# ethz-tb/orcAI

Measured on AMD Instinct MI355X. Metric: audio_seconds_per_s, higher is better.
Workload: dtype f32; 1 GPU; orcai-V1 predict, 1 h synthetic recording @48 kHz, 1833 snippets; parallelism=independent recordings x1

## Files before the change

orcai_amd/csrc/model_fwd.hip:

```cpp
#include <hip/hip_runtime.h>
#include <type_traits>

#include <cstdint>

#include "lds_dma.h"
#include "orcai_hip.h"
#include "zero_fill.h"

__attribute__((visibility("hidden"))) int lstm_wide_fwd_launch(const float* xz, const float* Uw, int B, int T, int units, float* out, float* gates, float* cstate, void* stream);

int g_orcai_lstm_split = 1;

namespace {

typedef float f32x4 __attribute__((ext_vector_type(4)));

__device__ __forceinline__ f32x4 mfma16(float a, float b, f32x4 c) { return __builtin_amdgcn_mfma_f32_16x16x4f32(a, b, c, 0, 0, 0); }


__device__ __forceinline__ void xcd_remap(int& bx, int& by) {
  const unsigned nbx = gridDim.x, total = nbx * gridDim.y;
  const unsigned L = blockIdx.y * nbx + blockIdx.x;
  const unsigned k = L & 7u, q = total >> 3, r = total & 7u;
  const unsigned Lp = k * q + (k < r ? k : r) + (L >> 3);
// ... 1572 lines not shown
#pragma unroll
      for (int m = 0; m < MT; ++m) acc[m][t] = mfma16(afrag[m], d[t], acc[m][t]);
  }

#pragma unroll
  for (int t = 0; t < 4; ++t) {
#pragma unroll
    for (int m = 0; m < MT; ++m) {
      const int oq = m * 4 + lk;
      const int e0 = VERT ? 2 * t : 3 * t;
      float mx[4] = {v[e0][m].x, v[e0][m].y, v[e0][m].z, v[e0][m].w};
#pragma unroll
      for (int dy = 1; dy < 3; ++dy) {
        mx[0] = fmaxf(mx[0], v[e0 + dy][m].x); mx[1] = fmaxf(mx[1], v[e0 + dy][m].y);
        mx[2] = fmaxf(mx[2], v[e0 + dy][m].z); mx[3] = fmaxf(mx[3], v[e0 + dy][m].w);
      }
      if (oidx[t] >= 0 && oq < CQ) {
        float o[4];
#pragma unroll
        for (int r = 0; r < 4; ++r) o[r] = (oq * 4 + r < C) ? mx[r] + (acc[m][t][r] + br_r[m][r]) : 0.0f;
        if (!SCATTER) {
          reinterpret_cast<float4*>(out)[((int64_t)b * CQ + oq) * plane_o + oidx[t]] = make_float4(o[0], o[1], o[2], o[3]);
        } else {
          const int orow = oidx[t] / WPo - R, ocol = oidx[t] - (orow + R) * WPo;
          const int rr = rm.base + b * rm.img_step + orow;
          if ((orow >= rm.r_lo || rr == orow) && orow < rm.r_hi) {
            const float4 val = make_float4(o[0], o[1], o[2], o[3]);
#pragma unroll
            for (int fi = 0; fi < kRowFamilies; ++fi) {
              if (fi >= rm.nfam) break;
              const RowFamily& fm = rm.f[fi];
              const int rel = rr - fm.offset - fm.keep_lo;
              if (rel < 0) continue;
              const int jhi = rel / fm.period;
              const int64_t plane_d = (int64_t)(fm.Hd + 2 * R) * WPo;
#pragma unroll
              for (int d = 0; d < 2; ++d) {
                const int j = jhi - d, y = rr - fm.offset - j * fm.period;
                if (j >= 0 && j < fm.count && y < fm.keep_hi)
                  reinterpret_cast<float4*>(fm.out)[((int64_t)j * CQ + oq) * plane_d + (int64_t)(y + R) * WPo + ocol] = val;
              }
            }
          }
        }
      }
    }
    if (t + DEPTH < 4) {
      load_tile(t + DEPTH);
      __builtin_amdgcn_sched_barrier(0);
    }
  }
}

constexpr int GP = 128 + 16;

constexpr int GBK = 32;

__global__ __launch_bounds__(256) void gemm_kernel(const float* __restrict__ A, const float* __restrict__ Bm, const float* __restrict__ bias,
                                                    const float* __restrict__ scale, const float* __restrict__ shift, float* __restrict__ C,
                                                    int M, int N, int K, int act, int vec) {
  __shared__ __attribute__((aligned(16))) float As[GBK][GP];
  __shared__ __attribute__((aligned(16))) float Bs[GBK][GP];
  const int tid = threadIdx.x, lane = tid & 63, wave = tid >> 6;
  const int wm = wave >> 1, wn = wave & 1;
  const int lk = lane >> 4, lj = lane & 15;
  const int64_t m0 = (int64_t)blockIdx.y * 128;
  const int n0 = blockIdx.x * 128;
  f32x4 acc[4][4];
#pragma unroll
  for (int i = 0; i < 4; ++i)
#pragma unroll
    for (int j = 0; j < 4; ++j) acc[i][j] = (f32x4){0.f, 0.f, 0.f, 0.f};

  float4 ra[4], rb[4];
  auto fetch = [&](int k0) {
#pragma unroll
    for (int g = 0; g < 4; ++g) {
      const int f = tid + 256 * g;
      {
        const int64_t m = m0 + (f & 127);
        const int k = k0 + (f >> 7) * 4;
        float v[4] = {0.f, 0.f, 0.f, 0.f};
        if (m < M) {
          const float* p = A + m * K + k;
          if (vec && k + 3 < K) {
            const float4 t = *reinterpret_cast<const float4*>(p);
            v[0] = t.x; v[1] = t.y; v[2] = t.z; v[3] = t.w;
          } else {
#pragma unroll
            for (int e = 0; e < 4; ++e) v[e] = (k + e < K) ? p[e] : 0.0f;
          }
        }
        ra[g] = make_float4(v[0], v[1], v[2], v[3]);
      }
      {
        const int k = k0 + (f >> 5), n = n0 + (f & 31) * 4;
        float v[4] = {0.f, 0.f, 0.f, 0.f};
        if (k < K) {
          const float* p = Bm + (int64_t)k * N + n;
          if (vec && n + 3 < N) {
            const float4 t = *reinterpret_cast<const float4*>(p);
            v[0] = t.x; v[1] = t.y; v[2] = t.z; v[3] = t.w;
          } else {
#pragma unroll
            for (int e = 0; e < 4; ++e) v[e] = (n + e < N) ? p[e] : 0.0f;
          }
        }
        rb[g] = make_float4(v[0], v[1], v[2], v[3]);
      }
    }
  };
  fetch(0);
  for (int k0 = 0; k0 < K; k0 += GBK) {
    __syncthreads();
#pragma unroll
    for (int g = 0; g < 4; ++g) {
      const int f = tid + 256 * g;
      const int m = f & 127, k = (f >> 7) * 4;
      As[k][m] = ra[g].x; As[k + 1][m] = ra[g].y; As[k + 2][m] = ra[g].z; As[k + 3][m] = ra[g].w;
      *reinterpret_cast<float4*>(&Bs[f >> 5][(f & 31) * 4]) = rb[g];
    }
    __syncthreads();
    if (k0 + GBK < K) fetch(k0 + GBK);
#pragma unroll
    for (int kk = 0; kk < GBK / 4; ++kk) {
      float a[4], bq[4];
#pragma unroll
      for (int i = 0; i < 4; ++i) a[i] = As[kk * 4 + lk][wm * 64 + i * 16 + lj];
#pragma unroll
      for (int j = 0; j < 4; ++j) bq[j] = Bs[kk * 4 + lk][wn * 64 + j * 16 + lj];
#pragma unroll
      for (int i = 0; i < 4; ++i)
#pragma unroll
        for (int j = 0; j < 4; ++j) acc[i][j] = mfma16(a[i], bq[j], acc[i][j]);
    }
  }
#pragma unroll
  for (int i = 0; i < 4; ++i)
#pragma unroll
    for (int r = 0; r < 4; ++r) {
      const int64_t m = m0 + wm * 64 + i * 16 + lk * 4 + r;
      if (m >= M) continue;
#pragma unroll
      for (int j = 0; j < 4; ++j) {
        const int n = n0 + wn * 64 + j * 16 + lj;
        if (n >= N) continue;
        float v = acc[i][j][r] + (bias ? bias[n] : 0.0f);
        if (act == 1) v = fmaxf(v, 0.0f);
        if (scale) v = fmaf(v, scale[n], shift[n]);
        C[m * N + n] = v;
      }
    }
}

__device__ __forceinline__ float sigmoidf_(float x) { return __builtin_amdgcn_rcpf(1.0f + __expf(-x)); }
__device__ __forceinline__ float tanhf_(float x) { return fmaf(-2.0f, __builtin_amdgcn_rcpf(__expf(2.0f * x) + 1.0f), 1.0f); }

__device__ __forceinline__ float dpp_xor8(float v) {
  return __uint_as_float(__builtin_amdgcn_update_dpp(0u, __float_as_uint(v), 0x128 , 0xf, 0xf, true));
}
template <class StoreState>
__device__ __forceinline__ void lstm_gate_stage(const float (&z0)[4], const float (&z1)[4], float (&cst)[4], int lj, StoreState store_state) {
  const bool low = lj < 8;
  const float m1 = low ? 2.0f : -1.0f;
  float a0[4], a1[4];
#pragma unroll
  for (int r = 0; r < 4; ++r) {
    a0[r] = sigmoidf_(z0[r]);
    const float rc = __builtin_amdgcn_rcpf(__expf(m1 * z1[r]) + 1.0f);
    a1[r] = low ? fmaf(-2.0f, rc, 1.0f) : rc;
  }
#pragma unroll
  for (int j = 0; j < 2; ++j) {
    const float got0 = dpp_xor8(low ? a0[2 + j] : a0[j]), got1 = dpp_xor8(low ? a1[2 + j] : a1[j]);
    const float gi = low ? a0[j] : got0, gf = low ? got0 : a0[2 + j];
    const float gg = low ? a1[j] : got1, go = low ? got1 : a1[2 + j];
    const float c = gf * cst[j] + gi * gg;
    const float h = go * tanhf_(c);
    cst[j] = c;
    store_state(low ? j : 2 + j, h);
  }
}

template <int U>
__global__ __launch_bounds__(U * 8) void lstm_kernel(const float* __restrict__ xz , const float* __restrict__ Uw ,
                                                      int B, int T, float* __restrict__ out ) {
  constexpr int KSTEPS = U / 4, HP = U + 2;
  __shared__ float hbuf[2][16][HP];
  const int tid = threadIdx.x, lane = tid & 63, wave = tid >> 6;
  const int lk = lane >> 4, lj = lane & 15;
  const int dir = blockIdx.y;
  const int b0 = blockIdx.x * 16;
  const float* Ud = Uw + (int64_t)dir * U * 4 * U;

  float ufrag[2][KSTEPS];
#pragma unroll
  for (int nt = 0; nt < 2; ++nt)
#pragma unroll
    for (int kk = 0; kk < KSTEPS; ++kk) ufrag[nt][kk] = Ud[(int64_t)(kk * 4 + lk) * (4 * U) + wave * 32 + nt * 16 + lj];

  for (int i = tid; i < 2 * 16 * HP; i += U * 8) (&hbuf[0][0][0])[i] = 0.0f;
  float cst[4] = {0.f, 0.f, 0.f, 0.f};
  __syncthreads();

  const int unit = wave * 8 + (lj & 7);
// ... 774 lines not shown
    hipLaunchKernelGGL((pool_res_add_x_kernel<MT, true, true>), vgrid, dim3(256), 0, st, s, prev, C, Cp, H, W, WP, R, Ho, Wo, WPo, tot_h / 2, wr, br, out, compact, \
                       vtasks, mg, ntc, rm);                                                                                                                     \
  else                                                                                                                                                           \
    hipLaunchKernelGGL((pool_res_add_x_kernel<MT, false, true>), grid, dim3(256), 0, st, s, prev, C, Cp, H, W, WP, R, Ho, Wo, WPo, tot_h / 2, wr, br, out, compact, \
                       tasks, mg, 0, rm)
  switch ((C + 15) / 16) {
    case 1: ORCAI_POOL_SCATTER(1); break;
    case 2: ORCAI_POOL_SCATTER(2); break;
    case 3: ORCAI_POOL_SCATTER(3); break;
    case 4: ORCAI_POOL_SCATTER(4); break;
  }
#undef ORCAI_POOL_SCATTER
  return (int)hipGetLastError();
}

int orcai_pool_res_add_scatter(const float* s, const float* prev, int B, int C, int Cp, int H, int W, int ksize, const float* wr, const float* br, float* out,
                               int xpooled, int Hd, int nsnip, int period, int base, int img_step, int r_lo, int r_hi, int keep_lo, int keep_hi,
                               void* stream) {
  if (!s || !prev || !wr || !br || !out || B <= 0 || C <= 0 || Cp <= 0 || H <= 0 || W <= 0 || nsnip <= 0 || period <= 0) return ORCAI_E_BADARG;
  if (xpooled & ~3) return ORCAI_E_BADARG;
  if (keep_lo < 0 || keep_hi > Hd || keep_lo >= keep_hi || Hd != 2 * period || base < 0 || img_step < 0) return ORCAI_E_BADARG;
  RowMap rm{};
  rm.base = base;
  rm.img_step = img_step;
  rm.r_lo = r_lo;
  rm.r_hi = r_hi;
  rm.nfam = 1;
  rm.f[0] = RowFamily{out, Hd, period, 0, nsnip, keep_lo, keep_hi};
  return pool_res_scatter_launch(s, prev, B, C, Cp, H, W, ksize, wr, br, xpooled, rm, stream);
}

int orcai_pool_res_add_scatter_families(const float* s, const float* prev, int B, int C, int Cp, int H, int W, int ksize, const float* wr, const float* br,
                                        int xpooled, int base, int img_step, int r_lo, int r_hi, const orcai_row_family* fams, int nfam, void* stream) {
  if (!s || !prev || !wr || !br || !fams || B <= 0 || C <= 0 || Cp <= 0 || H <= 0 || W <= 0 || nfam <= 0) return ORCAI_E_BADARG;
  if ((xpooled & ~3) || base < 0 || img_step < 0) return ORCAI_E_BADARG;
  if (nfam > kRowFamilies) return ORCAI_E_UNSUPPORTED;
  RowMap rm{};
  rm.base = base;
  rm.img_step = img_step;
  rm.r_lo = r_lo;
  rm.r_hi = r_hi;
  rm.nfam = nfam;
  for (int i = 0; i < nfam; ++i) {
    const orcai_row_family& f = fams[i];
    if (!f.out || f.Hd <= 0 || f.period <= 0 || f.count <= 0 || f.offset < 0 || f.keep_lo < 0 || f.keep_hi > f.Hd || f.keep_lo >= f.keep_hi)
      return ORCAI_E_BADARG;
    if (f.keep_hi - f.keep_lo > 2 * f.period) return ORCAI_E_UNSUPPORTED;
    if ((int64_t)f.offset + (int64_t)(f.count - 1) * f.period + f.Hd >= (1ll << 31)) return ORCAI_E_UNSUPPORTED;
    rm.f[i] = RowFamily{f.out, f.Hd, f.period, f.offset, f.count, f.keep_lo, f.keep_hi};
  }
  return pool_res_scatter_launch(s, prev, B, C, Cp, H, W, ksize, wr, br, xpooled, rm, stream);
}

int orcai_gemm_bias_act(const float* A, const float* Bm, const float* bias, const float* scale, const float* shift, float* C, int64_t M, int N,
                        int K, int act, void* stream) {
  if (!A || !Bm || !C || M <= 0 || N <= 0 || K <= 0 || (scale && !shift)) return ORCAI_E_BADARG;
  dim3 grid((N + 127) / 128, (unsigned)((M + 127) / 128));
  const int vec = (((uintptr_t)A | (uintptr_t)Bm) % 16 == 0 && K % 4 == 0 && N % 4 == 0) ? 1 : 0;
  hipLaunchKernelGGL(gemm_kernel, grid, dim3(256), 0, (hipStream_t)stream, A, Bm, bias, scale, shift, C, (int)M, N, K, act, vec);
  return (int)hipGetLastError();
}

int orcai_lstm_split(int on) {
  const int prev = g_orcai_lstm_split;
  if (on >= 0) g_orcai_lstm_split = on ? 1 : 0;
  return prev;
}

int orcai_lstm_recurrent(const float* xz, const float* Uw, int B, int T, int units, float* out, void* stream) {
  if (!xz || !Uw || !out || B <= 0 || T <= 0) return ORCAI_E_BADARG;
  if (units < 32 || units > 256 || units % 32) return ORCAI_E_UNSUPPORTED;
  if (units > 128) return lstm_wide_fwd_launch(xz, Uw, B, T, units, out, nullptr, nullptr, stream);
  dim3 grid((B + 15) / 16, 2);
  hipStream_t st = (hipStream_t)stream;
  if (g_orcai_lstm_split) {
    switch (units) {
      case 128: hipLaunchKernelGGL(lstm_split_kernel<128>, grid, dim3(1024), 0, st, xz, Uw, B, T, out); break;
      case 64: hipLaunchKernelGGL(lstm_split_kernel<64>, grid, dim3(512), 0, st, xz, Uw, B, T, out); break;
      case 96: hipLaunchKernelGGL(lstm_split_kernel<96>, grid, dim3(768), 0, st, xz, Uw, B, T, out); break;
      case 32: hipLaunchKernelGGL(lstm_split_kernel<32>, grid, dim3(256), 0, st, xz, Uw, B, T, out); break;
      default: return ORCAI_E_UNSUPPORTED;
    }
    return (int)hipGetLastError();
  }
  switch (units) {
    case 128: hipLaunchKernelGGL(lstm_kernel<128>, grid, dim3(1024), 0, st, xz, Uw, B, T, out); break;
    case 64: hipLaunchKernelGGL(lstm_kernel<64>, grid, dim3(512), 0, st, xz, Uw, B, T, out); break;
    case 96: hipLaunchKernelGGL(lstm_kernel<96>, grid, dim3(768), 0, st, xz, Uw, B, T, out); break;
    case 32: hipLaunchKernelGGL(lstm_kernel<32>, grid, dim3(256), 0, st, xz, Uw, B, T, out); break;
    default: return ORCAI_E_UNSUPPORTED;
  }
  return (int)hipGetLastError();
}

int orcai_dense_sigmoid(const float* x, const float* w, const float* bias, int64_t M, int K, int N, float* out, void* stream) {
  if (!x || !w || !bias || !out || M <= 0 || K <= 0 || N <= 0) return ORCAI_E_BADARG;
  if (N > 64) return ORCAI_E_UNSUPPORTED;
  if (N > 8) {
    const dim3 grid((unsigned)((M + 31) / 32), (unsigned)((N + 15) / 16));
    if ((K & 3) == 0 && (reinterpret_cast<uintptr_t>(x) & 15) == 0)
      hipLaunchKernelGGL(dense_sigmoid_wide_kernel<true>, grid, dim3(256), 0, (hipStream_t)stream, x, w, bias, M, K, N, out);
    else
      hipLaunchKernelGGL(dense_sigmoid_wide_kernel<false>, grid, dim3(256), 0, (hipStream_t)stream, x, w, bias, M, K, N, out);
    return (int)hipGetLastError();
  }
  if ((K & 3) == 0 && (reinterpret_cast<uintptr_t>(x) & 15) == 0)
    hipLaunchKernelGGL(dense_sigmoid_rows_kernel, dim3((unsigned)((M + 31) / 32)), dim3(256), 0, (hipStream_t)stream, x, w, bias, M, K, N, out);
  else
    hipLaunchKernelGGL(dense_sigmoid_kernel, dim3((unsigned)((M + 255) / 256)), dim3(256), 0, (hipStream_t)stream, x, w, bias, M, K, N, out);
  return (int)hipGetLastError();
}

// ... 17 lines not shown
```

include/orcai_hip.h:

```cpp
#ifndef ORCAI_HIP_H
#define ORCAI_HIP_H

#include <stddef.h>
#include <stdint.h>

#ifdef __cplusplus
extern "C" {
#endif

#define ORCAI_E_BADARG (-1)
#define ORCAI_E_UNSUPPORTED (-2)

const char* orcai_version(void);


size_t orcai_frontend_workspace_bytes(void);

int orcai_frontend_reset(void* workspace, void* stream);

int orcai_pcm_decode(const void* frames, int64_t n_frames, int channels, int channel, int format, float* out, void* stream);

int orcai_pcm_decode_planar(const void* frames, int64_t n_frames, int channels, int format, float* out, int64_t stride, void* stream);

int orcai_resample_polyphase(const float* x, int64_t n_in, float* out, int64_t n_out, int L, int M, const float* table, int ntaps, void* stream);
// ... 16 lines not shown

int orcai_crop_transpose(const float* in_ft, int64_t n_freq, int64_t n_frames, int f_lo, int f_hi, float* out_tf, void* stream);

int orcai_frontend_stats_host(const void* workspace, float stats_host[6], void* stream);

int orcai_make_spectrogram(const float* pcm, int64_t n_samples, int n_fft, int hop, int64_t n_frames, int k_crop,
                           int64_t rank_lo, int64_t rank_hi, float top_db, float* out, void* workspace, void* stream);

int orcai_frontend_stats_dev(const void* workspace, float* stats_dev, void* stream);

int orcai_spectrogram_bwd(const float* pcm, int64_t n_samples, int n_fft, int hop, int64_t n_frames, int k_crop, const float* gout,
                          const float* stats_dev, float top_db, float* dpcm, void* stream);



int orcai_padded_width(int W, int ksize);

int orcai_sepconv_tile_mode(int mode);

int orcai_entry_windows(int windows_per_wave);

int orcai_entry_tile(int waves);

int orcai_conv0_bn_relu(const float* in, int64_t snippet_stride, int B, int H, int W, int ksize, const float* w, const float* scale,
                        const float* shift, float* out, void* stream);

int orcai_conv0_sepconv(const float* in, int64_t snippet_stride, int B, int H, int W, const float* w0, const float* scale0, const float* shift0,
                        const float* dw, const float* pw, const float* scale, const float* shift, int Cout, int relu_out, float* out, float* prev_sub,
                        void* stream);

int orcai_sepconv_bn(const float* in, int B, int Cin, int H, int W, int ksize, int relu_in, const float* dw, const float* pw, const float* scale,
                     const float* shift, int Cout, int relu_out, int out_layout, float* out, void* stream);

int orcai_pool_res_add(const float* s, const float* prev, int B, int C, int Cp, int H, int W, int ksize, const float* wr, const float* br,
                       float* out, int xpooled, void* stream);
int orcai_pool_res_add_scatter(const float* s, const float* prev, int B, int C, int Cp, int H, int W, int ksize, const float* wr, const float* br,
                               float* out, int xpooled, int Hd, int nsnip, int period, int base, int img_step, int r_lo, int r_hi, int keep_lo,
                               int keep_hi, void* stream);
#define ORCAI_ROW_FAMILIES 4
typedef struct {
  float* out;
  int Hd, period, offset, count, keep_lo, keep_hi;
} orcai_row_family;
int orcai_pool_res_add_scatter_families(const float* s, const float* prev, int B, int C, int Cp, int H, int W, int ksize, const float* wr,
                                        const float* br, int xpooled, int base, int img_step, int r_lo, int r_hi, const orcai_row_family* fams,
                                        int nfam, void* stream);
int orcai_sepconv_pool_res(const float* in, const float* prev, int B, int Cin, int C, int Cp, int H, int W, int ksize, int relu_in, const float* dw, const float* pw,
                           const float* scale, const float* shift, int relu_out, const float* wr, const float* br, float* out, int prev_compact, void* stream);
int orcai_pool_fused(int nt);
int orcai_pool_vertical(int on);

int orcai_gemm_bias_act(const float* A, const float* Bm, const float* bias, const float* scale, const float* shift, float* C, int64_t M, int N,
                        int K, int act, void* stream);

int orcai_lstm_recurrent(const float* xz, const float* Uw, int B, int T, int units, float* out, void* stream);

int orcai_dense_sigmoid(const float* x, const float* w, const float* bias, int64_t M, int K, int N, float* out, void* stream);

int orcai_overlap_average(const float* pred, int n, int P, int L, int step, int64_t S, double* agg, double* cnt, void* stream);

int orcai_overlap_average_ragged(const float* pred, int P, int L, int step, const int64_t* table, int R, int64_t S_total, double* agg, double* cnt,
                                 void* stream);


int orcai_gemm_strided(const float* A, int64_t sam, int64_t sak, const float* B, int64_t sbk, int64_t sbn, float* C, int M, int N, int K, float alpha,
                       int accumulate, const float* Wreg, float beta_w, void* stream);

int orcai_colsum(const float* x, int M, int C, float* out, int accumulate, void* stream);

int orcai_bn_rows_stats(const float* x, int M, int cols, int C, float* mean, float* var, void* stream);
int orcai_bn_rows_apply(const float* x, int M, int cols, int C, const float* mean, const float* var, const float* gamma, const float* beta, float eps,
                        int relu, float* y, void* stream);
int orcai_bn_rows_bwd(const float* dy, const float* x, int M, int cols, int C, const float* mean, const float* var, const float* gamma, const float* beta,
                      float eps, int relu, float* dbeta, float* dgamma, float* dx, void* stream);

int orcai_dropout_mask(float* mask, int64_t n, uint64_t seed, float keep, void* stream);
int orcai_mask_scale(const float* x, const float* mask, float scale, int64_t n, float* y, void* stream);
int orcai_relu_bwd(const float* dy, const float* y, int64_t n, float* dx, void* stream);

int orcai_masked_bce(const float* p, const float* y, int64_t n, float mask_value, double* acc3, float* dz, void* stream);
int orcai_masked_bce_w(const float* p, const float* y, int64_t n, float mask_value, double* acc3, float* dz, const float* loss_weight, float grad_scale,
                       void* stream);
int orcai_l2_value(const float* w, int64_t n, float lambda, double* out, void* stream);

int orcai_adam_step(float* w, const float* g, float* m, float* v, int64_t n, float lr, float b1, float b2, float eps, int step, float gscale, void* stream);

int orcai_lstm_split(int on);
int orcai_lstm_train_fwd(const float* xz, const float* Uw, int B, int T, int units, float* out, float* gates, float* cstate, void* stream);
int orcai_h_lstm_train_fwd(const float* xz, const float* Uw, int B, int T, int units, float* out, float* gates, float* cstate, void* stream);
int orcai_h_lstm_bwd(const float* dH, const float* gates, const float* cstate, const float* Uw, int B, int T, int units, float* dxz, void* stream);
int orcai_lstm_bwd(const float* dH, const float* gates, const float* cstate, const float* Uw, int B, int T, int units, float* dxz, void* stream);
int orcai_lstm_hprev(const float* h, int B, int T, int units, float* hprev, void* stream);

int orcai_conv0_affine(const float* in, int64_t snippet_stride, int B, int H, int W, int ksize, const float* w, const float* scale, const float* shift,
                       int relu, float* out, void* stream);

int orcai_freq_mean_bwd(const float* dfm, int64_t M, int W, int C, float* dfeat, void* stream);
int orcai_conv1d_bwd(const float* x, const float* w, const float* dz, int B, int T, int C, int K, int L, float* dW, float* dx, void* stream);

int orcai_gather_snippets(const float* store, const int64_t* row_starts, int B, int rows, int cols, float* out, void* stream);
int orcai_downsample_labels(const float* labels, const int64_t* row_starts, int B, int rows, int L, int factor, float* out, void* stream);

int orcai_freq_mean(const float* feat, int64_t M, int W, int C, float* out, void* stream);
int orcai_conv1d_sigmoid(const float* x, const float* w, const float* bias, int B, int T, int C, int K, int L, float* out, void* stream);

int orcai_sepconv_planes(const float* in, int B, int Cin, int H, int W, int ksize_planes, int ktap, int relu_in, const float* dw, const float* pw,
// ... 188 lines not shown
```

orcai_amd/_native.py:

```python

from __future__ import annotations

import ctypes as C
from pathlib import Path

LIB_PATH = Path(__file__).resolve().parent / "liborcai_hip.so"

_lib = None

c_i64 = C.c_int64
c_f32p = C.c_void_p

class UnpackDesc(C.Structure):

    _fields_ = [("src", C.c_void_p), ("ld_src", C.c_int), ("col_off", C.c_int), ("rows", C.c_int), ("G", C.c_void_p), ("W", C.c_void_p), ("l2g", C.c_float)]


class RowFamily(C.Structure):

    _fields_ = [("out", C.c_void_p), ("Hd", C.c_int), ("period", C.c_int), ("offset", C.c_int), ("count", C.c_int), ("keep_lo", C.c_int), ("keep_hi", C.c_int)]


_SIGNATURES = {
    "orcai_version": (C.c_char_p, []),
    "orcai_frontend_workspace_bytes": (C.c_size_t, []),
    "orcai_frontend_reset": (C.c_int, [C.c_void_p, C.c_void_p]),
    "orcai_stft_db": (C.c_int, [C.c_void_p, c_i64, C.c_int, C.c_int, c_i64, C.c_int, C.c_void_p, C.c_void_p, C.c_void_p]),
    "orcai_stft_occupancy": (C.c_int, []),
    "orcai_hist_level1": (C.c_int, [C.c_void_p, c_i64, C.c_void_p, C.c_void_p]),
    "orcai_quantile_select": (C.c_int, [C.c_void_p, c_i64, c_i64, c_i64, C.c_void_p, C.c_void_p]),
    "orcai_frontend_finalize": (C.c_int, [C.c_int, C.c_float, C.c_void_p, C.c_void_p]),
    "orcai_clip_normalize": (C.c_int, [C.c_void_p, c_i64, C.c_void_p, C.c_void_p]),
    "orcai_db_reference": (C.c_int, [C.c_void_p, c_i64, C.c_void_p, C.c_void_p]),
    "orcai_crop_transpose": (C.c_int, [C.c_void_p, c_i64, c_i64, C.c_int, C.c_int, C.c_void_p, C.c_void_p]),
    "orcai_frontend_stats_host": (C.c_int, [C.c_void_p, C.POINTER(C.c_float), C.c_void_p]),
    "orcai_conv0_bn_relu": (C.c_int, [C.c_void_p, c_i64, C.c_int, C.c_int, C.c_int, C.c_int, C.c_void_p, C.c_void_p, C.c_void_p, C.c_void_p, C.c_void_p]),
    "orcai_sepconv_bn": (C.c_int, [C.c_void_p, C.c_int, C.c_int, C.c_int, C.c_int, C.c_int, C.c_int, C.c_void_p, C.c_void_p, C.c_void_p, C.c_void_p, C.c_int, C.c_int, C.c_int, C.c_void_p, C.c_void_p]),
    "orcai_pool_res_add": (C.c_int, [C.c_void_p, C.c_void_p, C.c_int, C.c_int, C.c_int, C.c_int, C.c_int, C.c_int, C.c_void_p, C.c_void_p, C.c_void_p, C.c_int, C.c_void_p]),
    "orcai_pool_res_add_scatter": (C.c_int, [C.c_void_p, C.c_void_p] + [C.c_int] * 6 + [C.c_void_p] * 3 + [C.c_int] * 10 + [C.c_void_p]),
    "orcai_pool_res_add_scatter_families": (C.c_int, [C.c_void_p, C.c_void_p] + [C.c_int] * 6 + [C.c_void_p] * 2 + [C.c_int] * 5 + [C.c_void_p, C.c_int, C.c_void_p]),
    "orcai_padded_width": (C.c_int, [C.c_int, C.c_int]),
    "orcai_sepconv_tile_mode": (C.c_int, [C.c_int]),
    "orcai_entry_windows": (C.c_int, [C.c_int]),
    "orcai_entry_tile": (C.c_int, [C.c_int]),
    "orcai_conv0_sepconv": (C.c_int, [C.c_void_p, C.c_int64, C.c_int, C.c_int, C.c_int] + [C.c_void_p] * 7 + [C.c_int, C.c_int, C.c_void_p, C.c_void_p, C.c_void_p]),
    "orcai_gemm_bias_act": (C.c_int, [C.c_void_p, C.c_void_p, C.c_void_p, C.c_void_p, C.c_void_p, C.c_void_p, c_i64, C.c_int, C.c_int, C.c_int, C.c_void_p]),
    "orcai_lstm_recurrent": (C.c_int, [C.c_void_p, C.c_void_p, C.c_int, C.c_int, C.c_int, C.c_void_p, C.c_void_p]),
    "orcai_dense_sigmoid": (C.c_int, [C.c_void_p, C.c_void_p, C.c_void_p, c_i64, C.c_int, C.c_int, C.c_void_p, C.c_void_p]),
    "orcai_overlap_average": (C.c_int, [C.c_void_p, C.c_int, C.c_int, C.c_int, C.c_int, c_i64, C.c_void_p, C.c_void_p, C.c_void_p]),
    "orcai_gemm_strided": (C.c_int, [C.c_void_p, c_i64, c_i64, C.c_void_p, c_i64, c_i64, C.c_void_p, C.c_int, C.c_int, C.c_int, C.c_float, C.c_int, C.c_void_p, C.c_float, C.c_void_p]),
    "orcai_colsum": (C.c_int, [C.c_void_p, C.c_int, C.c_int, C.c_void_p, C.c_int, C.c_void_p]),
    "orcai_bn_rows_stats": (C.c_int, [C.c_void_p, C.c_int, C.c_int, C.c_int, C.c_void_p, C.c_void_p, C.c_void_p]),
    "orcai_bn_rows_apply": (C.c_int, [C.c_void_p, C.c_int, C.c_int, C.c_int, C.c_void_p, C.c_void_p, C.c_void_p, C.c_void_p, C.c_float, C.c_int, C.c_void_p, C.c_void_p]),
    "orcai_bn_rows_bwd": (C.c_int, [C.c_void_p, C.c_void_p, C.c_int, C.c_int, C.c_int, C.c_void_p, C.c_void_p, C.c_void_p, C.c_void_p, C.c_float, C.c_int, C.c_void_p, C.c_void_p, C.c_void_p, C.c_void_p]),
    "orcai_dropout_mask": (C.c_int, [C.c_void_p, c_i64, C.c_uint64, C.c_float, C.c_void_p]),
    "orcai_mask_scale": (C.c_int, [C.c_void_p, C.c_void_p, C.c_float, c_i64, C.c_void_p, C.c_void_p]),
    "orcai_relu_bwd": (C.c_int, [C.c_void_p, C.c_void_p, c_i64, C.c_void_p, C.c_void_p]),
    "orcai_masked_bce": (C.c_int, [C.c_void_p, C.c_void_p, c_i64, C.c_float, C.c_void_p, C.c_void_p, C.c_void_p]),
    "orcai_masked_bce_w": (C.c_int, [C.c_void_p, C.c_void_p, c_i64, C.c_float, C.c_void_p, C.c_void_p, C.c_void_p, C.c_float, C.c_void_p]),
    "orcai_l2_value": (C.c_int, [C.c_void_p, c_i64, C.c_float, C.c_void_p, C.c_void_p]),
    "orcai_adam_step": (C.c_int, [C.c_void_p, C.c_void_p, C.c_void_p, C.c_void_p, c_i64, C.c_float, C.c_float, C.c_float, C.c_float, C.c_int, C.c_float, C.c_void_p]),
    "orcai_lstm_split": (C.c_int, [C.c_int]),
    "orcai_lstm_train_fwd": (C.c_int, [C.c_void_p, C.c_void_p, C.c_int, C.c_int, C.c_int, C.c_void_p, C.c_void_p, C.c_void_p, C.c_void_p]),
    "orcai_h_lstm_train_fwd": (C.c_int, [C.c_void_p, C.c_void_p, C.c_int, C.c_int, C.c_int, C.c_void_p, C.c_void_p, C.c_void_p, C.c_void_p]),
    "orcai_lstm_bwd": (C.c_int, [C.c_void_p, C.c_void_p, C.c_void_p, C.c_void_p, C.c_int, C.c_int, C.c_int, C.c_void_p, C.c_void_p]),
    "orcai_h_lstm_bwd": (C.c_int, [C.c_void_p, C.c_void_p, C.c_void_p, C.c_void_p, C.c_int, C.c_int, C.c_int, C.c_void_p, C.c_void_p]),
    "orcai_lstm_hprev": (C.c_int, [C.c_void_p, C.c_int, C.c_int, C.c_int, C.c_void_p, C.c_void_p]),
    "orcai_conv0_affine": (C.c_int, [C.c_void_p, c_i64, C.c_int, C.c_int, C.c_int, C.c_int, C.c_void_p, C.c_void_p, C.c_void_p, C.c_int, C.c_void_p, C.c_void_p]),
    "orcai_gather_snippets": (C.c_int, [C.c_void_p, C.c_void_p, C.c_int, C.c_int, C.c_int, C.c_void_p, C.c_void_p]),
    "orcai_downsample_labels": (C.c_int, [C.c_void_p, C.c_void_p] + [C.c_int] * 4 + [C.c_void_p, C.c_void_p]),
    "orcai_freq_mean_bwd": (C.c_int, [C.c_void_p, C.c_int64, C.c_int, C.c_int, C.c_void_p, C.c_void_p]),
    "orcai_conv1d_bwd": (C.c_int, [C.c_void_p] * 3 + [C.c_int] * 5 + [C.c_void_p] * 3),
    "orcai_bn_bwd_pointwise": (C.c_int, [C.c_void_p, C.c_void_p] + [C.c_int] * 5 + [C.c_void_p] * 4 + [C.c_float, C.c_int, C.c_void_p, C.c_int] + [C.c_void_p] * 3 + [C.c_int] + [C.c_void_p] * 3),
    "orcai_pw_wgrad_tiles": (C.c_int, [C.c_int]),
    "orcai_bn_bwd_pointwise_wgrad": (C.c_int, [C.c_void_p] * 3 + [C.c_int] * 5 + [C.c_void_p] * 4 + [C.c_float, C.c_int, C.c_void_p, C.c_int] + [C.c_void_p] * 3 + [C.c_int] + [C.c_void_p] * 3 + [c_i64, C.c_void_p]),
    "orcai_h_bn_bwd_pointwise_wgrad": (C.c_int, [C.c_void_p] * 3 + [C.c_int] * 5 + [C.c_void_p] * 4 + [C.c_float, C.c_int, C.c_void_p, C.c_int] + [C.c_void_p] * 3 + [C.c_int] + [C.c_void_p] * 3 + [c_i64, C.c_void_p]),
    "orcai_pool_res_add_bn": (C.c_int, [C.c_void_p, C.c_void_p] + [C.c_int] * 6 + [C.c_void_p] * 3 + [C.c_int] + [C.c_void_p] * 4 + [C.c_float, C.c_void_p]),
    "orcai_pool_bwd_bn": (C.c_int, [C.c_void_p, C.c_void_p] + [C.c_int] * 5 + [C.c_void_p] * 4 + [C.c_float, C.c_void_p, C.c_void_p]),
    "orcai_pool_bwd_bn_bias": (C.c_int, [C.c_void_p, C.c_void_p] + [C.c_int] * 5 + [C.c_void_p] * 4 + [C.c_float] + [C.c_void_p] * 4),
    "orcai_h_pool_bwd_bn_bias": (C.c_int, [C.c_void_p, C.c_void_p] + [C.c_int] * 5 + [C.c_void_p] * 4 + [C.c_float] + [C.c_void_p] * 4),
    "orcai_conv0_bn_bwd": (C.c_int, [C.c_void_p, C.c_int64, C.c_void_p, C.c_void_p] + [C.c_int] * 4 + [C.c_void_p] * 4 + [C.c_float] + [C.c_void_p] * 5),
    "orcai_conv0_stats": (C.c_int, [C.c_void_p, C.c_int64] + [C.c_int] * 4 + [C.c_void_p] * 5),
    "orcai_conv0_affine_bn": (C.c_int, [C.c_void_p, C.c_int64] + [C.c_int] * 4 + [C.c_void_p] * 7 + [C.c_float, C.c_int, C.c_void_p, C.c_void_p]),
    "orcai_conv0_bn_bwd_x": (C.c_int, [C.c_void_p, C.c_int64, C.c_void_p] + [C.c_int] * 4 + [C.c_void_p] * 6 + [C.c_float] + [C.c_void_p] * 5 + [c_i64, C.c_void_p]),
    "orcai_pack_weights": (C.c_int, [C.c_void_p, C.c_void_p, C.c_int, C.c_void_p, C.c_void_p]),
    "orcai_freq_mean": (C.c_int, [C.c_void_p, C.c_int64, C.c_int, C.c_int, C.c_void_p, C.c_void_p]),
    "orcai_conv1d_sigmoid": (C.c_int, [C.c_void_p] * 3 + [C.c_int] * 5 + [C.c_void_p, C.c_void_p]),
    "orcai_sepconv_planes": (C.c_int, [C.c_void_p] + [C.c_int] * 7 + [C.c_void_p] * 4 + [C.c_int] * 5 + [C.c_void_p, C.c_void_p]),
    "orcai_sepconv_planes_u": (C.c_int, [C.c_void_p] + [C.c_int] * 7 + [C.c_void_p] * 4 + [C.c_int] * 5 + [C.c_void_p, C.c_void_p, C.c_void_p]),
    "orcai_sepconv_planes_stats": (C.c_int, [C.c_void_p] + [C.c_int] * 5 + [C.c_void_p] * 4 + [C.c_int] + [C.c_void_p] * 4),
    "orcai_dw_wgrad_march": (C.c_int, [C.c_int]),
    "orcai_pool_vertical": (C.c_int, [C.c_int]),
    "orcai_pool_fused": (C.c_int, [C.c_int]),
    "orcai_sepconv_pool_res": (C.c_int, [C.c_void_p] * 2 + [C.c_int] * 8 + [C.c_void_p] * 4 + [C.c_int] + [C.c_void_p] * 3 + [C.c_int, C.c_void_p]),
    "orcai_dw_bwd_fused": (C.c_int, [C.c_void_p, C.c_void_p] + [C.c_int] * 5 + [C.c_void_p] * 3 + [C.c_int] + [C.c_void_p] * 4 + [C.c_float, C.c_int, C.c_void_p, C.c_void_p]),
    "orcai_dw_bwd_fused_conv0": (C.c_int, [C.c_void_p, C.c_int64, C.c_void_p] + [C.c_int] * 3 + [C.c_void_p] * 9 + [C.c_float, C.c_void_p, C.c_void_p, C.c_void_p]),
    "orcai_conv0_bn_bwd_x_ready": (C.c_int, [C.c_void_p, C.c_int64, C.c_void_p] + [C.c_int] * 4 + [C.c_void_p] * 6 + [C.c_float] + [C.c_void_p] * 5 + [c_i64, C.c_void_p]),
    "orcai_conv0_bn_bwd_dx": (C.c_int, [C.c_void_p, C.c_int64, C.c_void_p] + [C.c_int] * 4 + [C.c_void_p] * 6 + [C.c_float] + [C.c_void_p] * 3),
    "orcai_conv0_stats_march": (C.c_int, [C.c_void_p, C.c_int64] + [C.c_int] * 3 + [C.c_void_p] * 5),
# ... 137 lines not shown
```

Before: 153,100 audio-s/s.

## Double-buffer GEMM LDS tiles with float4 layout and vectorized epilogue

Rewrites the generic fp32 MFMA GEMM to keep two LDS buffers, so the next K-tile is staged and fetched while the current one is computed, with a single barrier per iteration. Shared tiles are now float4-packed, which lets the A and B fragments be read with wide LDS loads. Boundary loads use clamped addresses instead of branches. The epilogue stores float4 per thread with templated activation and scale paths, and each thread's columns are remapped to be contiguous. LDS use doubles and the tail-handling logic becomes more intricate.

```diff
diff --git a/orcai_amd/csrc/model_fwd.hip b/orcai_amd/csrc/model_fwd.hip
--- a/orcai_amd/csrc/model_fwd.hip
+++ b/orcai_amd/csrc/model_fwd.hip
@@ -1648,15 +1648,45 @@
   }
 }
 
-constexpr int GP = 128 + 16;
-
 constexpr int GBK = 32;
 
-__global__ __launch_bounds__(256) void gemm_kernel(const float* __restrict__ A, const float* __restrict__ Bm, const float* __restrict__ bias,
-                                                    const float* __restrict__ scale, const float* __restrict__ shift, float* __restrict__ C,
-                                                    int M, int N, int K, int act, int vec) {
-  __shared__ __attribute__((aligned(16))) float As[GBK][GP];
-  __shared__ __attribute__((aligned(16))) float Bs[GBK][GP];
+template <int ACT, bool SCALE, bool CVEC>
+__device__ __forceinline__ void gemm_store(const f32x4 (&acc)[4][4], const float (&bv)[4], const float (&sv)[4], const float (&hv)[4], float* __restrict__ C,
+                                           int64_t mbase, int M, int N, int n, int lk) {
+#pragma unroll
+  for (int i = 0; i < 4; ++i)
+#pragma unroll
+    for (int r = 0; r < 4; ++r) {
+      const int64_t m = mbase + i * 16 + lk * 4 + r;
+      float v[4];
+#pragma unroll
+      for (int j = 0; j < 4; ++j) {
+        v[j] = acc[i][j][r] + bv[j];
+        if (ACT == 1) v[j] = fmaxf(v[j], 0.0f);
+        if (SCALE) v[j] = fmaf(v[j], sv[j], hv[j]);
+      }
+      float* p = C + m * N + n;
+      if (CVEC) {
+        if (m < M && n < N) *reinterpret_cast<float4*>(p) = make_float4(v[0], v[1], v[2], v[3]);
+      } else {
+#pragma unroll
+        for (int j = 0; j < 4; ++j)
+          if (m < M && n + j < N) p[j] = v[j];
+      }
+    }
+}
+
+template <int ACT, bool SCALE>
+__device__ __forceinline__ void gemm_store(const f32x4 (&acc)[4][4], const float (&bv)[4], const float (&sv)[4], const float (&hv)[4], float* __restrict__ C,
+                                           int64_t mbase, int M, int N, int n, int lk, int cvec) {
+  if (cvec) gemm_store<ACT, SCALE, true>(acc, bv, sv, hv, C, mbase, M, N, n, lk);
+  else gemm_store<ACT, SCALE, false>(acc, bv, sv, hv, C, mbase, M, N, n, lk);
+}
+
+template <bool VEC>
+__device__ __forceinline__ void gemm_tile(float4 (&As)[2][GBK / 4][128], float4 (&Bs)[2][GBK][32], const float* __restrict__ A, const float* __restrict__ Bm,
+                                          const float* __restrict__ bias, const float* __restrict__ scale, const float* __restrict__ shift,
+                                          float* __restrict__ C, int M, int N, int K, int act, int cvec) {
   const int tid = threadIdx.x, lane = tid & 63, wave = tid >> 6;
   const int wm = wave >> 1, wn = wave & 1;
   const int lk = lane >> 4, lj = lane & 15;
@@ -1668,85 +1698,101 @@
 #pragma unroll
     for (int j = 0; j < 4; ++j) acc[i][j] = (f32x4){0.f, 0.f, 0.f, 0.f};
 
-  float4 ra[4], rb[4];
+  float ra[4][4], rb[4][4];
+  const float* arow = A + (m0 + (tid & 127) < M ? m0 + (tid & 127) : (int64_t)M - 1) * K;
   auto fetch = [&](int k0) {
 #pragma unroll
     for (int g = 0; g < 4; ++g) {
-      const int f = tid + 256 * g;
-      {
-        const int64_t m = m0 + (f & 127);
-        const int k = k0 + (f >> 7) * 4;
-        float v[4] = {0.f, 0.f, 0.f, 0.f};
-        if (m < M) {
-          const float* p = A + m * K + k;
-          if (vec && k + 3 < K) {
-            const float4 t = *reinterpret_cast<const float4*>(p);
-            v[0] = t.x; v[1] = t.y; v[2] = t.z; v[3] = t.w;
-          } else {
-#pragma unroll
-            for (int e = 0; e < 4; ++e) v[e] = (k + e < K) ? p[e] : 0.0f;
-          }
+      const int ka = k0 + (tid >> 7) * 16 + 4 * g, kb = k0 + (tid >> 5) + 8 * g, n = n0 + (tid & 31) * 4;
+      if (VEC) {
+        const float4 ta = *reinterpret_cast<const float4*>(arow + min(ka, K - 4));
+        const float4 tb = *reinterpret_cast<const float4*>(Bm + (int64_t)min(kb, K - 1) * N + min(n, N - 4));
+        ra[g][0] = ta.x; ra[g][1] = ta.y; ra[g][2] = ta.z; ra[g][3] = ta.w;
+        rb[g][0] = tb.x; rb[g][1] = tb.y; rb[g][2] = tb.z; rb[g][3] = tb.w;
+      } else {
+        const float* brow = Bm + (int64_t)min(kb, K - 1) * N;
+#pragma unroll
+        for (int e = 0; e < 4; ++e) {
+          const float va = arow[min(ka + e, K - 1)], vb = brow[min(n + e, N - 1)];
+          ra[g][e] = ka + e < K ? va : 0.0f;
+          rb[g][e] = kb < K ? vb : 0.0f;
         }
-        ra[g] = make_float4(v[0], v[1], v[2], v[3]);
-      }
-      {
-        const int k = k0 + (f >> 5), n = n0 + (f & 31) * 4;
-        float v[4] = {0.f, 0.f, 0.f, 0.f};
-        if (k < K) {
-          const float* p = Bm + (int64_t)k * N + n;
-          if (vec && n + 3 < N) {
-            const float4 t = *reinterpret_cast<const float4*>(p);
-            v[0] = t.x; v[1] = t.y; v[2] = t.z; v[3] = t.w;
-          } else {
-#pragma unroll
-            for (int e = 0; e < 4; ++e) v[e] = (n + e < N) ? p[e] : 0.0f;
-          }
+      }
+    }
+  };
+  auto stage = [&](int slot) {
+#pragma unroll
+    for (int q = 0; q < 4; ++q) As[slot][(tid >> 7) * 4 + q][tid & 127] = make_float4(ra[0][q], ra[1][q], ra[2][q], ra[3][q]);
+#pragma unroll
+    for (int g = 0; g < 4; ++g) Bs[slot][(tid >> 5) + 8 * g][tid & 31] = make_float4(rb[g][0], rb[g][1], rb[g][2], rb[g][3]);
+  };
+  auto compute = [&](int slot, int nst) {
+#pragma unroll
+    for (int J = 0; J < GBK / 16; ++J) {
+      if (J * 4 >= nst) break;
+      float4 a[4];
+#pragma unroll
+      for (int i = 0; i < 4; ++i) a[i] = As[slot][J * 4 + lk][wm * 64 + i * 16 + lj];
+#pragma unroll
+      for (int jj = 0; jj < 4; ++jj) {
+        if (J * 4 + jj >= nst) break;
+        const float4 b = Bs[slot][(J * 4 + jj) * 4 + lk][wn * 16 + lj];
+        const float bq[4] = {b.x, b.y, b.z, b.w};
+#pragma unroll
+        for (int i = 0; i < 4; ++i) {
+          const float ai = jj == 0 ? a[i].x : jj == 1 ? a[i].y : jj == 2 ? a[i].z : a[i].w;
+#pragma unroll
+          for (int j = 0; j < 4; ++j) acc[i][j] = mfma16(ai, bq[j], acc[i][j]);
         }
-        rb[g] = make_float4(v[0], v[1], v[2], v[3]);
       }
     }
   };
+
+  const int nsteps = (K + 3) >> 2, ntiles = (nsteps + 7) >> 3;
   fetch(0);
-  for (int k0 = 0; k0 < K; k0 += GBK) {
+  stage(0);
+  if (ntiles > 1) fetch(GBK);
+  for (int t = 0; t < ntiles - 2; ++t) {
     __syncthreads();
-#pragma unroll
-    for (int g = 0; g < 4; ++g) {
-      const int f = tid + 256 * g;
-      const int m = f & 127, k = (f >> 7) * 4;
-      As[k][m] = ra[g].x; As[k + 1][m] = ra[g].y; As[k + 2][m] = ra[g].z; As[k + 3][m] = ra[g].w;
-      *reinterpret_cast<float4*>(&Bs[f >> 5][(f & 31) * 4]) = rb[g];
-    }
+    stage((t + 1) & 1);
+    fetch((t + 2) * GBK);
+    __builtin_amdgcn_sched_barrier(0);
+    compute(t & 1, 8);
+  }
+  if (ntiles > 1) {
     __syncthreads();
-    if (k0 + GBK < K) fetch(k0 + GBK);
-#pragma unroll
-    for (int kk = 0; kk < GBK / 4; ++kk) {
-      float a[4], bq[4];
-#pragma unroll
-      for (int i = 0; i < 4; ++i) a[i] = As[kk * 4 + lk][wm * 64 + i * 16 + lj];
-#pragma unroll
-      for (int j = 0; j < 4; ++j) bq[j] = Bs[kk * 4 + lk][wn * 64 + j * 16 + lj];
-#pragma unroll
-      for (int i = 0; i < 4; ++i)
-#pragma unroll
-        for (int j = 0; j < 4; ++j) acc[i][j] = mfma16(a[i], bq[j], acc[i][j]);
-    }
-  }
-#pragma unroll
-  for (int i = 0; i < 4; ++i)
-#pragma unroll
-    for (int r = 0; r < 4; ++r) {
-      const int64_t m = m0 + wm * 64 + i * 16 + lk * 4 + r;
-      if (m >= M) continue;
-#pragma unroll
-      for (int j = 0; j < 4; ++j) {
-        const int n = n0 + wn * 64 + j * 16 + lj;
-        if (n >= N) continue;
-        float v = acc[i][j][r] + (bias ? bias[n] : 0.0f);
-        if (act == 1) v = fmaxf(v, 0.0f);
-        if (scale) v = fmaf(v, scale[n], shift[n]);
-        C[m * N + n] = v;
-      }
-    }
+    stage((ntiles - 1) & 1);
+    compute(ntiles & 1, 8);
+  }
+  __syncthreads();
+  compute((ntiles - 1) & 1, nsteps - (ntiles - 1) * 8);
+
+  const int n = n0 + wn * 64 + lj * 4;
+  float bv[4], sv[4], hv[4];
+#pragma unroll
+  for (int j = 0; j < 4; ++j) {
+    const bool in = n + j < N;
+    bv[j] = (bias && in) ? bias[n + j] : 0.0f;
+    sv[j] = (scale && in) ? scale[n + j] : 0.0f;
+    hv[j] = (scale && in) ? shift[n + j] : 0.0f;
+  }
+  const int64_t mbase = m0 + wm * 64;
+  if (scale) {
+    if (act == 1) gemm_store<1, true>(acc, bv, sv, hv, C, mbase, M, N, n, lk, cvec);
+    else gemm_store<0, true>(acc, bv, sv, hv, C, mbase, M, N, n, lk, cvec);
+  } else {
+    if (act == 1) gemm_store<1, false>(acc, bv, sv, hv, C, mbase, M, N, n, lk, cvec);
+    else gemm_store<0, false>(acc, bv, sv, hv, C, mbase, M, N, n, lk, cvec);
+  }
+}
+
+__global__ __launch_bounds__(256) void gemm_kernel(const float* __restrict__ A, const float* __restrict__ Bm, const float* __restrict__ bias,
+                                                    const float* __restrict__ scale, const float* __restrict__ shift, float* __restrict__ C,
+                                                    int M, int N, int K, int act, int vec) {
+  __shared__ float4 As[2][GBK / 4][128];
+  __shared__ float4 Bs[2][GBK][32];
+  if (vec & 1) gemm_tile<true>(As, Bs, A, Bm, bias, scale, shift, C, M, N, K, act, vec >> 1);
+  else gemm_tile<false>(As, Bs, A, Bm, bias, scale, shift, C, M, N, K, act, vec >> 1);
 }
 
 __device__ __forceinline__ float sigmoidf_(float x) { return __builtin_amdgcn_rcpf(1.0f + __expf(-x)); }
@@ -2632,7 +2678,8 @@
   if (!A || !Bm || !C || M <= 0 || N <= 0 || K <= 0 || (scale && !shift)) return ORCAI_E_BADARG;
   dim3 grid((N + 127) / 128, (unsigned)((M + 127) / 128));
   const int vec = (((uintptr_t)A | (uintptr_t)Bm) % 16 == 0 && K % 4 == 0 && N % 4 == 0) ? 1 : 0;
-  hipLaunchKernelGGL(gemm_kernel, grid, dim3(256), 0, (hipStream_t)stream, A, Bm, bias, scale, shift, C, (int)M, N, K, act, vec);
+  const int cvec = ((uintptr_t)C % 16 == 0 && N % 4 == 0) ? 2 : 0;
+  hipLaunchKernelGGL(gemm_kernel, grid, dim3(256), 0, (hipStream_t)stream, A, Bm, bias, scale, shift, C, (int)M, N, K, act, vec | cvec);
   return (int)hipGetLastError();
 }
 
```

Result: no change. 154,300 audio-s/s, median of 6 (+0.8%).

## Rework GEMM kernel with XCD block remap, float4 epilogue stores, and ablation variants

Applied to the files above, without the earlier changes.

Replaces the default GEMM kernel with a templated body that remaps block indices across XCDs, drops the padded shared-memory layout, and changes the MFMA output row mapping so each lane holds four consecutive columns. This allows float4 vectorized C stores and vectorized bias/scale/shift loads. A runtime variant switch keeps the old kernel and ablation variants (no remap, double buffering, scalar stores) for comparison. The GEMM likely matters little next to the conv and LSTM stages, and the unpadded layout may add LDS bank conflicts.

```diff
diff --git a/include/orcai_hip.h b/include/orcai_hip.h
--- a/include/orcai_hip.h
+++ b/include/orcai_hip.h
@@ -92,6 +92,7 @@
 
 int orcai_gemm_bias_act(const float* A, const float* Bm, const float* bias, const float* scale, const float* shift, float* C, int64_t M, int N,
                         int K, int act, void* stream);
+int orcai_gemm_variant(int v);
 
 int orcai_lstm_recurrent(const float* xz, const float* Uw, int B, int T, int units, float* out, void* stream);
 
diff --git a/orcai_amd/_native.py b/orcai_amd/_native.py
--- a/orcai_amd/_native.py
+++ b/orcai_amd/_native.py
@@ -45,6 +45,7 @@
     "orcai_entry_tile": (C.c_int, [C.c_int]),
     "orcai_conv0_sepconv": (C.c_int, [C.c_void_p, C.c_int64, C.c_int, C.c_int, C.c_int] + [C.c_void_p] * 7 + [C.c_int, C.c_int, C.c_void_p, C.c_void_p, C.c_void_p]),
     "orcai_gemm_bias_act": (C.c_int, [C.c_void_p, C.c_void_p, C.c_void_p, C.c_void_p, C.c_void_p, C.c_void_p, c_i64, C.c_int, C.c_int, C.c_int, C.c_void_p]),
+    "orcai_gemm_variant": (C.c_int, [C.c_int]),
     "orcai_lstm_recurrent": (C.c_int, [C.c_void_p, C.c_void_p, C.c_int, C.c_int, C.c_int, C.c_void_p, C.c_void_p]),
     "orcai_dense_sigmoid": (C.c_int, [C.c_void_p, C.c_void_p, C.c_void_p, c_i64, C.c_int, C.c_int, C.c_void_p, C.c_void_p]),
     "orcai_overlap_average": (C.c_int, [C.c_void_p, C.c_int, C.c_int, C.c_int, C.c_int, c_i64, C.c_void_p, C.c_void_p, C.c_void_p]),
diff --git a/orcai_amd/csrc/model_fwd.hip b/orcai_amd/csrc/model_fwd.hip
--- a/orcai_amd/csrc/model_fwd.hip
+++ b/orcai_amd/csrc/model_fwd.hip
@@ -1652,7 +1652,7 @@
 
 constexpr int GBK = 32;
 
-__global__ __launch_bounds__(256) void gemm_kernel(const float* __restrict__ A, const float* __restrict__ Bm, const float* __restrict__ bias,
+__global__ __launch_bounds__(256) void gemm_kernel_v1(const float* __restrict__ A, const float* __restrict__ Bm, const float* __restrict__ bias,
                                                     const float* __restrict__ scale, const float* __restrict__ shift, float* __restrict__ C,
                                                     int M, int N, int K, int act, int vec) {
   __shared__ __attribute__((aligned(16))) float As[GBK][GP];
@@ -1747,6 +1747,176 @@
         C[m * N + n] = v;
       }
     }
+}
+
+constexpr int GQ = 128;
+
+template <bool REMAP, bool DBUF, bool WIDE>
+__device__ __forceinline__ void gemm_body(const float* __restrict__ A, const float* __restrict__ Bm, const float* __restrict__ bias,
+                                          const float* __restrict__ scale, const float* __restrict__ shift, float* __restrict__ C, int M, int N, int K,
+                                          int act, int flags) {
+  constexpr int NBUF = DBUF ? 2 : 1;
+  __shared__ __attribute__((aligned(16))) float As[NBUF][GBK][GQ];
+  __shared__ __attribute__((aligned(16))) float Bs[NBUF][GBK][GQ];
+  const int tid = threadIdx.x, lane = tid & 63, wave = tid >> 6;
+  const int wm = wave >> 1, wn = wave & 1;
+  const int lk = lane >> 4, lj = lane & 15;
+  const int vec = flags & 1;
+  int bx = blockIdx.x, by = blockIdx.y;
+  if (REMAP) xcd_remap(bx, by);
+  const int64_t m0 = (int64_t)by * 128;
+  const int n0 = bx * 128;
+  f32x4 acc[4][4];
+#pragma unroll
+  for (int i = 0; i < 4; ++i)
+#pragma unroll
+    for (int j = 0; j < 4; ++j) acc[i][j] = (f32x4){0.f, 0.f, 0.f, 0.f};
+
+  float4 ra[4], rb[4];
+  auto fetch = [&](int k0) {
+#pragma unroll
+    for (int g = 0; g < 4; ++g) {
+      const int f = tid + 256 * g;
+      {
+        const int64_t m = m0 + (f & 127);
+        const int k = k0 + (f >> 7) * 4;
+        float v[4] = {0.f, 0.f, 0.f, 0.f};
+        if (m < M) {
+          const float* p = A + m * K + k;
+          if (vec && k + 3 < K) {
+            const float4 t = *reinterpret_cast<const float4*>(p);
+            v[0] = t.x; v[1] = t.y; v[2] = t.z; v[3] = t.w;
+          } else {
+#pragma unroll
+            for (int e = 0; e < 4; ++e) v[e] = (k + e < K) ? p[e] : 0.0f;
+          }
+        }
+        ra[g] = make_float4(v[0], v[1], v[2], v[3]);
+      }
+      {
+        const int k = k0 + (f >> 5), n = n0 + (f & 31) * 4;
+        float v[4] = {0.f, 0.f, 0.f, 0.f};
+        if (k < K) {
+          const float* p = Bm + (int64_t)k * N + n;
+          if (vec && n + 3 < N) {
+            const float4 t = *reinterpret_cast<const float4*>(p);
+            v[0] = t.x; v[1] = t.y; v[2] = t.z; v[3] = t.w;
+          } else {
+#pragma unroll
+            for (int e = 0; e < 4; ++e) v[e] = (n + e < N) ? p[e] : 0.0f;
+          }
+        }
+        rb[g] = make_float4(v[0], v[1], v[2], v[3]);
+      }
+    }
+  };
+  auto stash = [&](int buf) {
+#pragma unroll
+    for (int g = 0; g < 4; ++g) {
+      const int f = tid + 256 * g;
+      const int m = f & 127, k = (f >> 7) * 4;
+      As[buf][k][m] = ra[g].x; As[buf][k + 1][m] = ra[g].y; As[buf][k + 2][m] = ra[g].z; As[buf][k + 3][m] = ra[g].w;
+      *reinterpret_cast<float4*>(&Bs[buf][f >> 5][(f & 31) * 4]) = rb[g];
+    }
+  };
+  auto mac = [&](int buf) {
+#pragma unroll
+    for (int kk = 0; kk < GBK / 4; ++kk) {
+      const float4 av = *reinterpret_cast<const float4*>(&As[buf][kk * 4 + lk][wm * 64 + 4 * lj]);
+      const float4 bv = *reinterpret_cast<const float4*>(&Bs[buf][kk * 4 + lk][wn * 64 + 4 * lj]);
+      const float a[4] = {av.x, av.y, av.z, av.w}, bq[4] = {bv.x, bv.y, bv.z, bv.w};
+#pragma unroll
+      for (int i = 0; i < 4; ++i)
+#pragma unroll
+        for (int j = 0; j < 4; ++j) acc[i][j] = mfma16(a[i], bq[j], acc[i][j]);
+    }
+  };
+  fetch(0);
+  if (DBUF) {
+    stash(0);
+    __syncthreads();
+    int buf = 0;
+    for (int k0 = 0; k0 < K; k0 += GBK, buf ^= 1) {
+      const bool more = k0 + GBK < K;
+      if (more) fetch(k0 + GBK);
+      mac(buf);
+      if (more) stash(buf ^ 1);
+      __syncthreads();
+    }
+  } else {
+    for (int k0 = 0; k0 < K; k0 += GBK) {
+      __syncthreads();
+      stash(0);
+      __syncthreads();
+      if (k0 + GBK < K) fetch(k0 + GBK);
+      mac(0);
+    }
+  }
+
+  const int nl = n0 + wn * 64 + 4 * lj;
+  float bi[4] = {0.f, 0.f, 0.f, 0.f}, sc[4] = {0.f, 0.f, 0.f, 0.f}, sh[4] = {0.f, 0.f, 0.f, 0.f};
+  if ((flags & 4) && nl < N) {
+    if (bias) { const float4 t = *reinterpret_cast<const float4*>(bias + nl); bi[0] = t.x; bi[1] = t.y; bi[2] = t.z; bi[3] = t.w; }
+    if (scale) {
+      const float4 t = *reinterpret_cast<const float4*>(scale + nl), u = *reinterpret_cast<const float4*>(shift + nl);
+      sc[0] = t.x; sc[1] = t.y; sc[2] = t.z; sc[3] = t.w;
+      sh[0] = u.x; sh[1] = u.y; sh[2] = u.z; sh[3] = u.w;
+    }
+  } else {
+#pragma unroll
+    for (int j = 0; j < 4; ++j)
+      if (nl + j < N) {
+        if (bias) bi[j] = bias[nl + j];
+        if (scale) { sc[j] = scale[nl + j]; sh[j] = shift[nl + j]; }
+      }
+  }
+  auto finish = [&](int i, int r, float (&v)[4]) {
+#pragma unroll
+    for (int j = 0; j < 4; ++j) {
+      v[j] = acc[i][j][r] + bi[j];
+      if (act == 1) v[j] = fmaxf(v[j], 0.0f);
+      if (scale) v[j] = fmaf(v[j], sc[j], sh[j]);
+    }
+  };
+  if (WIDE && (flags & 2)) {
+    if (nl >= N) return;
+#pragma unroll
+    for (int i = 0; i < 4; ++i)
+#pragma unroll
+      for (int r = 0; r < 4; ++r) {
+        const int64_t m = m0 + wm * 64 + lk * 16 + r * 4 + i;
+        if (m >= M) continue;
+        float v[4];
+        finish(i, r, v);
+        *reinterpret_cast<float4*>(C + m * N + nl) = make_float4(v[0], v[1], v[2], v[3]);
+      }
+    return;
+  }
+#pragma unroll
+  for (int i = 0; i < 4; ++i)
+#pragma unroll
+    for (int r = 0; r < 4; ++r) {
+      const int64_t m = m0 + wm * 64 + lk * 16 + r * 4 + i;
+      if (m >= M) continue;
+      float v[4];
+      finish(i, r, v);
+#pragma unroll
+      for (int j = 3; j >= 0; --j)
+        if (nl + j < N) C[m * N + nl + j] = v[j];
+    }
+}
+
+__global__ __launch_bounds__(256) void gemm_kernel(const float* __restrict__ A, const float* __restrict__ Bm, const float* __restrict__ bias,
+                                                    const float* __restrict__ scale, const float* __restrict__ shift, float* __restrict__ C,
+                                                    int M, int N, int K, int act, int flags) {
+  gemm_body<true, false, true>(A, Bm, bias, scale, shift, C, M, N, K, act, flags);
+}
+
+template <bool REMAP, bool DBUF, bool WIDE>
+__global__ __launch_bounds__(256) void gemm_ablate_kernel(const float* __restrict__ A, const float* __restrict__ Bm, const float* __restrict__ bias,
+                                                           const float* __restrict__ scale, const float* __restrict__ shift, float* __restrict__ C,
+                                                           int M, int N, int K, int act, int flags) {
+  gemm_body<REMAP, DBUF, WIDE>(A, Bm, bias, scale, shift, C, M, N, K, act, flags);
 }
 
 __device__ __forceinline__ float sigmoidf_(float x) { return __builtin_amdgcn_rcpf(1.0f + __expf(-x)); }
@@ -2627,12 +2797,35 @@
   return pool_res_scatter_launch(s, prev, B, C, Cp, H, W, ksize, wr, br, xpooled, rm, stream);
 }
 
+int g_gemm_variant = 1;
+
+int orcai_gemm_variant(int v) {
+  const int prev = g_gemm_variant;
+  if (v >= 0) g_gemm_variant = v > 4 ? 1 : v;
+  return prev;
+}
+
 int orcai_gemm_bias_act(const float* A, const float* Bm, const float* bias, const float* scale, const float* shift, float* C, int64_t M, int N,
                         int K, int act, void* stream) {
   if (!A || !Bm || !C || M <= 0 || N <= 0 || K <= 0 || (scale && !shift)) return ORCAI_E_BADARG;
   dim3 grid((N + 127) / 128, (unsigned)((M + 127) / 128));
   const int vec = (((uintptr_t)A | (uintptr_t)Bm) % 16 == 0 && K % 4 == 0 && N % 4 == 0) ? 1 : 0;
-  hipLaunchKernelGGL(gemm_kernel, grid, dim3(256), 0, (hipStream_t)stream, A, Bm, bias, scale, shift, C, (int)M, N, K, act, vec);
+  hipStream_t st = (hipStream_t)stream;
+  if (g_gemm_variant == 0) {
+    hipLaunchKernelGGL(gemm_kernel_v1, grid, dim3(256), 0, st, A, Bm, bias, scale, shift, C, (int)M, N, K, act, vec);
+    return (int)hipGetLastError();
+  }
+  const int wide = (N % 4 == 0 && (uintptr_t)C % 16 == 0) ? 2 : 0;
+  const int pvec = (N % 4 == 0 && ((uintptr_t)bias | (uintptr_t)scale | (uintptr_t)shift) % 16 == 0) ? 4 : 0;
+  const int flags = vec | wide | pvec;
+#define ORCAI_GEMM_LAUNCH(KERNEL) hipLaunchKernelGGL(KERNEL, grid, dim3(256), 0, st, A, Bm, bias, scale, shift, C, (int)M, N, K, act, flags)
+  switch (g_gemm_variant) {
+    case 2: ORCAI_GEMM_LAUNCH((gemm_ablate_kernel<false, false, true>)); break;
+    case 3: ORCAI_GEMM_LAUNCH((gemm_ablate_kernel<true, true, true>)); break;
+    case 4: ORCAI_GEMM_LAUNCH((gemm_ablate_kernel<true, false, false>)); break;
+    default: ORCAI_GEMM_LAUNCH(gemm_kernel); break;
+  }
+#undef ORCAI_GEMM_LAUNCH
   return (int)hipGetLastError();
 }
 
```

Measured after the change: 149,500 audio-s/s before, 150,200 audio-s/s after, median of 6. Within noise of the previous version (+0.5%).
